# imdea-software/legosnark

Measured on AMD Instinct MI355X. Metric: alt_bn128 G1 MSM point-scalar pairs/s at n=2^20, higher is better.
Workload: dtype u32 limbs (254-bit Montgomery integers)

## Files before the change

legosnark_amd/csrc/msm.hip:

```cpp
#include <hip/hip_runtime.h>
#include <stdint.h>
#include <stdio.h>
#include <stdlib.h>
#include <string.h>
#include <algorithm>
#include <type_traits>
#include <vector>

#include "curves.h"
#include "fp29x2l.h"
#include "fs29.h"
#include "glv.h"
#include "msm.h"
#include "msm_plan.h"

namespace lsa {


template <class F, int K>
__global__ __launch_bounds__(256) void k_normalize(const Jac<F> *__restrict__ in, Aff<F> *__restrict__ out, size_t n) {
    size_t t = (size_t)blockIdx.x * blockDim.x + threadIdx.x;
    size_t base = t * K;
    if (base >= n) return;
    F prod[K];
// ... 258 lines not shown
    const uint32_t *tb = tile_base + ((size_t)k * ntiles + t) * B;
    for (uint32_t x = threadIdx.x; x < B; x += 1024) base[x] = of[x] + tb[x];
    __syncthreads();
    const size_t lo = (size_t)t * SORT_TILE;
    const size_t hi = lo + SORT_TILE < n ? lo + SORT_TILE : n;
    const int32_t *dg = digits + (size_t)k * n;
    const uint16_t *rk = rank + (size_t)k * n;
    for (size_t i = lo + threadIdx.x; i < hi; i += 1024) {
        int32_t sd = dg[i];
        if (sd != 0) {
            uint32_t b = (uint32_t)(sd < 0 ? -sd : sd) - 1;
            uint32_t pt = i < npoints ? (uint32_t)i : ((uint32_t)(i - npoints) | 0x40000000u);
            pt += k * win_stride;
            entries[base[b] + rk[i]] = pt | (sd < 0 ? 0x80000000u : 0u);
        }
    }
}

__global__ __launch_bounds__(1024) void k_tile_scan_rows(const uint16_t *__restrict__ tile_hist, uint32_t Bc, uint32_t R, uint32_t pitch,
                                                         uint32_t *__restrict__ tile_base, uint32_t *__restrict__ hist,
                                                         uint32_t *__restrict__ zero1, uint32_t *__restrict__ zeron, uint32_t nzero) {
    __builtin_amdgcn_s_setprio(3);
    if (blockIdx.x == 0) {
        if (threadIdx.x == 0) *zero1 = 0;
        for (uint32_t x = threadIdx.x; x < nzero; x += 1024) zeron[x] = 0;
    }
    __shared__ uint32_t part[32][33];
    const unsigned lane = threadIdx.x & 63, wv = threadIdx.x >> 6;
    const unsigned bl = lane & 31, grp = 2 * wv + (lane >> 5);
    const uint32_t b = blockIdx.x * 32 + bl;
    const uint32_t per = (R + 31) / 32, r0 = grp * per, r1 = r0 + per < R ? r0 + per : R;
    constexpr uint32_t MAXPER = 16;
    uint32_t v[MAXPER];
    uint32_t sum = 0;
    const bool in_regs = per <= MAXPER;
    if (in_regs) {
#pragma unroll
        for (uint32_t j = 0; j < MAXPER; j++) {
            const uint32_t r = r0 + j;
            v[j] = (b < Bc && r < r1) ? tile_hist[(size_t)r * pitch + b] : 0u;
        }
#pragma unroll
        for (uint32_t j = 0; j < MAXPER; j++) sum += v[j];
    } else if (b < Bc) {
        for (uint32_t r = r0; r < r1; r++) sum += tile_hist[(size_t)r * pitch + b];
    }
    part[grp][bl] = sum;
// ... 152 lines not shown
    const size_t lo = (size_t)t * PART_TILE;
    const uint32_t fine_bits = cm.sh_hi;
    const uint32_t tlow = t & ((1u << (16 - fine_bits)) - 1);
    for (uint32_t j = 0; j < PART_TILE / 1024; j++) {
        const uint32_t il = threadIdx.x + j * 1024;
        const size_t i = lo + il;
        if (i >= n) break;
        const uint32_t seg = segment_of(segs, (uint32_t)i);
        wide_digits(scalars[i], pl, seg * B, [&](unsigned k, int32_t sd) {
            if (sd != 0) {
                const uint32_t b = (uint32_t)(sd < 0 ? -sd : sd) - 1;
                const uint32_t pos = atomicAdd(&lcur[cm.bin(b)], 1u);
                stage[pos] = (tlow << (16 + fine_bits)) | (cm.fine(b) << 16) | (k << 12) | (sd < 0 ? 0x800u : 0u) | il;
            }
        });
    }
    __syncthreads();
    for (uint32_t sg = threadIdx.x >> 5; sg < Bc; sg += 32) {
        const uint32_t a = lstart[sg], e = lstart[sg + 1], g = gdst[sg];
        for (uint32_t x = a + (lane & 31); x < e; x += 32) recs[g + (x - a)] = stage[x];
    }
}

__global__ __launch_bounds__(1024) void k_fine_sort_part(const uint32_t *__restrict__ recs, const uint32_t *__restrict__ offs_c,
                                                         const uint32_t *__restrict__ hist_c, const uint32_t *__restrict__ tile_base,
                                                         uint32_t pitch, uint32_t T, CoarseMap cm, SegList segs, uint32_t win_stride, uint32_t stage_cap,
                                                         uint32_t *__restrict__ entries, uint32_t *__restrict__ hist, uint32_t *__restrict__ offs) {
    __builtin_amdgcn_s_setprio(3);
    extern __shared__ __attribute__((aligned(16))) uint32_t sm[];
    __shared__ uint32_t wsum[16];
    const uint32_t sg = blockIdx.x, lo = offs_c[sg], ns = hist_c[sg];
    const uint32_t fine_bits = cm.sh_hi, FM = 1u << fine_bits, fmask = FM - 1, tbits = 16 - fine_bits;
    const uint32_t F = 1u << cm.bits(sg), bucket0 = cm.first(sg);
    uint32_t *cnt = sm, *cur = sm + FM, *col = sm + 2 * FM, *stage = col + T + 1;
    const unsigned lane = threadIdx.x & 63, wv = threadIdx.x >> 6;
    for (uint32_t x = threadIdx.x; x < F; x += 1024) cnt[x] = 0;
    for (uint32_t x = threadIdx.x; x < T; x += 1024) col[x] = tile_base[(size_t)x * pitch + sg];
    if (threadIdx.x == 0) col[T] = ns;
    auto scan_counters = [&]() {
        const uint32_t per = (F + 1023) >> 10, f0 = threadIdx.x * per;
        uint32_t sum = 0;
        for (uint32_t q = 0; q < per; q++) if (f0 + q < F) sum += cnt[f0 + q];
        uint32_t incl = sum;
#pragma unroll
        for (int d = 1; d < 64; d <<= 1) {
            const uint32_t u = __shfl_up(incl, d, 64);
            if ((int)lane >= d) incl += u;
        }
        if (lane == 63) wsum[wv] = incl;
        __syncthreads();
        uint32_t run = incl - sum;
        for (unsigned w = 0; w < wv; w++) run += wsum[w];
        for (uint32_t q = 0; q < per; q++) {
            if (f0 + q >= F) break;
            const uint32_t c = cnt[f0 + q];
            cur[f0 + q] = run;
            hist[(size_t)bucket0 + f0 + q] = c;
            offs[(size_t)bucket0 + f0 + q] = lo + run;
            run += c;
        }
    };
    auto entry_of = [&](uint32_t r, uint32_t p2) {
        uint32_t a = 0, e = (T + (1u << tbits) - 1) >> tbits;
        while (e - a > 1) {
            const uint32_t m = (a + e) >> 1;
            if (col[m << tbits] <= p2) a = m; else e = m;
        }
        const uint32_t i = ((a << tbits) | (r >> (16 + fine_bits))) * PART_TILE + (r & 0x7ffu);
        const uint32_t local = i - segs.off[segment_of(segs, i)];
        return (local + ((r >> 12) & 15u) * win_stride) | ((r & 0x800u) << 20);
    };
    if (ns <= stage_cap) {
        constexpr uint32_t NR = PART_STAGE / 1024;
        uint32_t r[NR];
#pragma unroll
        for (uint32_t u = 0; u < NR; u++) { const uint32_t p2 = threadIdx.x + u * 1024; r[u] = p2 < ns ? recs[lo + p2] : 0u; }
        __syncthreads();
        uint16_t rk[NR];
#pragma unroll
        for (uint32_t u = 0; u < NR; u++) {
            rk[u] = 0;
            if (threadIdx.x + u * 1024 < ns) rk[u] = (uint16_t)atomicAdd(&cnt[(r[u] >> 16) & fmask], 1u);
        }
        __syncthreads();
        scan_counters();
        __syncthreads();
#pragma unroll
        for (uint32_t u = 0; u < NR; u++) {
            const uint32_t p2 = threadIdx.x + u * 1024;
            if (p2 < ns) stage[cur[(r[u] >> 16) & fmask] + rk[u]] = entry_of(r[u], p2);
        }
        __syncthreads();
        for (uint32_t x = threadIdx.x; x < ns; x += 1024) entries[lo + x] = stage[x];
        return;
    }
    __syncthreads();
    constexpr uint32_t UNR = 8;
    for (uint32_t p0 = threadIdx.x; p0 < ns; p0 += 1024 * UNR) {
        uint32_t r[UNR];
#pragma unroll
        for (uint32_t u = 0; u < UNR; u++) { const uint32_t p2 = p0 + u * 1024; r[u] = p2 < ns ? recs[lo + p2] : 0u; }
#pragma unroll
        for (uint32_t u = 0; u < UNR; u++) if (p0 + u * 1024 < ns) (void)lds_inc_rank(cnt, (r[u] >> 16) & fmask);
    }
    __syncthreads();
    scan_counters();
    __syncthreads();
    for (uint32_t p0 = threadIdx.x; p0 < ns; p0 += 1024 * UNR) {
        uint32_t r[UNR];
#pragma unroll
        for (uint32_t u = 0; u < UNR; u++) { const uint32_t p2 = p0 + u * 1024; r[u] = p2 < ns ? recs[lo + p2] : 0u; }
#pragma unroll
        for (uint32_t u = 0; u < UNR; u++) {
            const uint32_t p2 = p0 + u * 1024;
            if (p2 >= ns) break;
            entries[lo + lds_inc_rank(cur, (r[u] >> 16) & fmask)] = entry_of(r[u], p2);
        }
    }
}

template <class Rec>
struct RecOps;
template <>
struct RecOps<uint64_t> {
    static constexpr uint32_t NF = 128;
    static __device__ __forceinline__ uint32_t fine(uint64_t r) { return (uint32_t)(r >> 32); }
    static __device__ __forceinline__ uint32_t entry(uint64_t r) { return (uint32_t)r; }
};
template <>
struct RecOps<uint32_t> {
// ... 21 lines not shown
        uint32_t incl = tot;
#pragma unroll
        for (int d = 1; d < 64; d <<= 1) {
            uint32_t t = __shfl_up(incl, d, 64);
            if ((int)threadIdx.x >= d) incl += t;
        }
        uint32_t ex = incl - tot;
#pragma unroll
        for (uint32_t q = 0; q < PER; q++) {
            cur[PER * threadIdx.x + q] = ex;
            hist[(size_t)bin * NF + PER * threadIdx.x + q] = c[q];
            offs[(size_t)bin * NF + PER * threadIdx.x + q] = lo + ex;
            ex += c[q];
        }
    }
    __syncthreads();
    for (uint32_t j = threadIdx.x; j < n; j += 1024) {
        const Rec r = recs[lo + j];
        const uint32_t pos = atomicAdd(&cur[O::fine(r)], 1u);
        entries[lo + pos] = O::entry(r);
    }
}

__device__ __forceinline__ uint32_t size_bin(uint32_t cnt, uint32_t bin_shift) { return ((cnt - 1) >> bin_shift) + 1; }
template <class C>
__global__ __launch_bounds__(256) void k_size_hist(const uint32_t *__restrict__ hist, uint32_t nb, uint32_t thr, uint32_t *__restrict__ bin_count,
                                                   uint32_t group_size, uint32_t bin_shift) {
    bin_count += (group_size ? (blockIdx.x * 2048u) / group_size : 0u) * SIZE_BINS;
    __shared__ uint32_t lcnt[SIZE_BINS];
    for (uint32_t t = threadIdx.x; t < SIZE_BINS; t += 256) lcnt[t] = 0;
    __syncthreads();
    const uint32_t base = blockIdx.x * 2048 + threadIdx.x;
#pragma unroll
    for (int j = 0; j < 8; j++) {
        uint32_t g = base + j * 256;
        if (g < nb) { uint32_t cnt = hist[g]; if (cnt > 0 && cnt <= thr) atomicAdd(&lcnt[size_bin(cnt, bin_shift)], 1u); }
    }
    __syncthreads();
    for (uint32_t t = threadIdx.x; t < SIZE_BINS; t += 256) if (lcnt[t]) atomicAdd(&bin_count[t], lcnt[t]);
}
__global__ __launch_bounds__(256) void k_size_scan(const uint32_t *__restrict__ bin_count, uint32_t *__restrict__ bin_start, uint32_t ngroups) {
    __shared__ uint32_t lds[4];
    uint32_t carry = 0;
    for (uint32_t gidx = 0; gidx < ngroups; gidx++) {
        const uint32_t *bc = bin_count + gidx * SIZE_BINS;
        uint32_t *bs = bin_start + gidx * SIZE_BINS;
        uint32_t v[4], s = 0;
#pragma unroll
        for (int j = 0; j < 4; j++) {
            int bin = (int)SIZE_BINS - 1 - (int)(threadIdx.x * 4 + j);
            v[j] = (bin >= 1) ? bc[bin] : 0;
            s += v[j];
        }
        uint32_t tot;
        uint32_t run = carry + block_exclusive_scan_256(s, lds, &tot);
#pragma unroll
        for (int j = 0; j < 4; j++) {
            int bin = (int)SIZE_BINS - 1 - (int)(threadIdx.x * 4 + j);
            if (bin >= 1) bs[bin] = run;
            run += v[j];
        }
        carry += tot;
    }
    if (threadIdx.x == 0) bin_start[0] = carry;
}
template <class C>
__global__ __launch_bounds__(256) void k_size_scatter(const uint32_t *__restrict__ hist, uint32_t nb, uint32_t thr, const uint32_t *__restrict__ bin_start,
                                                      uint32_t *__restrict__ bin_cursor, uint32_t *__restrict__ perm,
                                                      uint32_t *__restrict__ heavy_list, uint32_t *__restrict__ heavy_count,
                                                      typename C::Acc *__restrict__ buckets, uint32_t group_size, uint32_t bin_shift,
                                                      uint32_t split) {
    const uint32_t goff = (group_size ? (blockIdx.x * 2048u) / group_size : 0u) * SIZE_BINS;
    bin_start += goff;
    bin_cursor += goff;
    __shared__ uint32_t lcnt[SIZE_BINS];
    for (uint32_t t = threadIdx.x; t < SIZE_BINS; t += 256) lcnt[t] = 0;
    __syncthreads();
    const uint32_t base = blockIdx.x * 2048 + threadIdx.x;
    uint32_t cnt[8], rank[8];
#pragma unroll
    for (int j = 0; j < 8; j++) {
        uint32_t g = base + j * 256;
        cnt[j] = 0; rank[j] = 0;
        if (g < nb) {
            cnt[j] = hist[g];
            if (cnt[j] == 0) { for (uint32_t h = 0; h < split; h++) buckets[(size_t)g * split + h] = C::inf(); }
            else if (cnt[j] > thr) heavy_list[atomicAdd(heavy_count, 1u)] = g;
            else rank[j] = atomicAdd(&lcnt[size_bin(cnt[j], bin_shift)], 1u);
        }
    }
    __syncthreads();
    for (uint32_t t = threadIdx.x; t < SIZE_BINS; t += 256) {
        uint32_t c = lcnt[t];
        lcnt[t] = c ? atomicAdd(&bin_cursor[t], c) : 0;
    }
    __syncthreads();
#pragma unroll
    for (int j = 0; j < 8; j++) {
        uint32_t g = base + j * 256;
        if (g < nb && cnt[j] > 0 && cnt[j] <= thr) {
            const uint32_t bin = size_bin(cnt[j], bin_shift);
            perm[bin_start[bin] + lcnt[bin] + rank[j]] = g;
        }
    }
}

typedef uint32_t u32x4 __attribute__((ext_vector_type(4)));
template <class B> struct RawBase {
    static_assert(sizeof(B) % 16 == 0, "packed bases are whole 16-byte vectors");
    u32x4 q[sizeof(B) / 16];
};
template <class B>
__device__ __forceinline__ RawBase<B> load_base16(const B *__restrict__ p) {
    const u32x4 *src = reinterpret_cast<const u32x4 *>(p);
    RawBase<B> r;
#pragma unroll
    for (int i = 0; i < (int)(sizeof(B) / 16); i++) r.q[i] = src[i];
    return r;
}
template <class B>
__device__ __forceinline__ B packed_base(RawBase<B> r) {
    B b;
    uint32_t *dst = reinterpret_cast<uint32_t *>(&b);
#pragma unroll
    for (int i = 0; i < (int)(sizeof(B) / 16); i++) {
        asm("" : "+v"(r.q[i]));
// ... 42 lines not shown
            const typename C::Base b0 = packed_base(r0), b1 = packed_base(r1);
            cur = r0;
            if (j + ACC_SPLIT < cnt && C::head_ok(b0, b1)) {
                acc = C::template madd_head<ENDO>(b0, (v >> 31) != 0, ((v >> 30) & 1) != 0, b1, (vn >> 31) != 0, ((vn >> 30) & 1) != 0);
                j += 2 * ACC_SPLIT;
                v = v2;
                vn = v3;
                cur = r2;
            }
        } else {
            cur = base(v);
        }
        for (; j < cnt; j += ACC_SPLIT) {
            const uint32_t vnn = word(j + 2 * ACC_SPLIT);
            const RawBase<typename C::Base> nxt = base(vn);
            acc = C::template madd<ENDO>(acc, packed_base(cur), (v >> 31) != 0, ((v >> 30) & 1) != 0);
            v = vn;
            vn = vnn;
            cur = nxt;
        }
    }
    buckets[(size_t)g * ACC_SPLIT + part] = acc;
}
template <class C, uint32_t ACC_SPLIT>
__global__ __launch_bounds__(256) void k_accumulate(const typename C::Base *__restrict__ bases, const uint32_t *__restrict__ entries,
                                                    const uint32_t *__restrict__ offs, const uint32_t *__restrict__ hist,
                                                    const uint32_t *__restrict__ perm, const uint32_t *__restrict__ nperm,
                                                    typename C::Acc *__restrict__ buckets) {
    accumulate_body<C, ACC_SPLIT>(bases, entries, offs, hist, perm, nperm, buckets);
}
__global__ __launch_bounds__(256) __attribute__((amdgpu_waves_per_eu(2, 2))) void k_accumulate_g2_occ2(
    const CurveG2::Base *__restrict__ bases, const uint32_t *__restrict__ entries, const uint32_t *__restrict__ offs,
    const uint32_t *__restrict__ hist, const uint32_t *__restrict__ perm, const uint32_t *__restrict__ nperm, CurveG2::Acc *__restrict__ buckets) {
    accumulate_body<CurveG2, 1u>(bases, entries, offs, hist, perm, nperm, buckets);
}

__global__ __launch_bounds__(256) void k_accumulate_g2_pair(const AffPackedG2 *__restrict__ bases, const uint32_t *__restrict__ entries,
                                                            const uint32_t *__restrict__ offs, const uint32_t *__restrict__ hist,
                                                            const uint32_t *__restrict__ perm, const uint32_t *__restrict__ nperm,
                                                            XYZZ29x2 *__restrict__ buckets) {
    const uint32_t t = blockIdx.x * blockDim.x + threadIdx.x, pr = t >> 1, part = t & 1;
    if (pr >= *nperm) return;
    const uint32_t g = perm[pr];
    const uint32_t cnt = hist[g];
    const uint32_t *e = entries + offs[g];
    struct Half { uint32_t x[8], y[8]; };
    auto fetch = [&](uint32_t v) {
        const AffPackedG2 &b = bases[v & 0x3fffffffu];
        Half h;
#pragma unroll
        for (int i = 0; i < 8; i++) { h.x[i] = b.w[part][i]; h.y[i] = b.w[2 + part][i]; }
// ... 26 lines not shown
    A r;
    constexpr int NW = sizeof(A) / 4;
    const uint32_t *src = reinterpret_cast<const uint32_t *>(&p);
    uint32_t *dst = reinterpret_cast<uint32_t *>(&r);
#pragma unroll
    for (int i = 0; i < NW; i++) dst[i] = __shfl_down(src[i], delta, 64);
    return r;
}

enum TailKernel { TAIL_HEAVY, TAIL_REDUCE1_LANE, TAIL_REDUCE2_LANE };
template <class C, TailKernel K> struct PairedAdd { static constexpr bool value = false; };
template <> struct PairedAdd<CurveG1, TAIL_HEAVY> { static constexpr bool value = true; };
template <> struct PairedAdd<CurveG1, TAIL_REDUCE1_LANE> { static constexpr bool value = true; };

template <class C, bool PAIRED = false>
__device__ __forceinline__ typename C::Acc wave_sum(typename C::Acc v, unsigned lane) {
    for (unsigned d = 32; d >= 1; d >>= 1) {
        typename C::Acc t = shfl_down_acc(v, d);
        if (lane + d < 64) v = C::template add<PAIRED>(v, t);
    }
    return v;
}

__global__ __launch_bounds__(256) void k_heavy_plan(const uint32_t *__restrict__ hist, const uint32_t *__restrict__ heavy_list,
                                                    const uint32_t *__restrict__ heavy_count, uint32_t *__restrict__ chunk_off) {
    __shared__ uint32_t lds[4];
    __shared__ uint32_t s_chunk;
    const uint32_t nh = *heavy_count;
    uint32_t carry = 0;
    for (uint32_t base = 0; base < nh; base += 256) {
        uint32_t h = base + threadIdx.x;
        uint32_t tot;
        (void)block_exclusive_scan_256(h < nh ? hist[heavy_list[h]] : 0, lds, &tot);
        carry += tot;
    }
    if (threadIdx.x == 0) {
        uint32_t chunk = HEAVY_CHUNK;
        while (chunk < 4096u && carry / (2 * chunk) >= 2048u) chunk *= 2;
        s_chunk = chunk;
    }
    __syncthreads();
    const uint32_t chunk = s_chunk;
    carry = 0;
    for (uint32_t base = 0; base < nh; base += 256) {
        uint32_t h = base + threadIdx.x;
        uint32_t v = h < nh ? (hist[heavy_list[h]] + chunk - 1) / chunk : 0;
        uint32_t tot;
        uint32_t ex = block_exclusive_scan_256(v, lds, &tot);
        if (h < nh) chunk_off[h] = carry + ex;
        carry += tot;
    }
    if (threadIdx.x == 0) { chunk_off[nh] = carry; chunk_off[nh + 1] = chunk; }
}

template <class C>
__global__ __launch_bounds__(64) void k_accumulate_heavy(const typename C::Base *__restrict__ bases, const uint32_t *__restrict__ entries,
                                                         const uint32_t *__restrict__ offs, const uint32_t *__restrict__ hist,
                                                         const uint32_t *__restrict__ heavy_list, const uint32_t *__restrict__ heavy_count,
                                                         const uint32_t *__restrict__ chunk_off, typename C::Acc *__restrict__ partials) {
    const uint32_t nh = *heavy_count;
    if (nh == 0) return;
    const uint32_t total = chunk_off[nh], chunk = chunk_off[nh + 1];
    const unsigned lane = threadIdx.x;
    for (uint32_t v = blockIdx.x; v < total; v += gridDim.x) {
        uint32_t lo = 0, hi = nh;
        while (hi - lo > 1) { uint32_t mid = (lo + hi) >> 1; if (chunk_off[mid] <= v) lo = mid; else hi = mid; }
        const uint32_t g = heavy_list[lo];
        const uint32_t cnt = hist[g];
        const uint32_t start = (v - chunk_off[lo]) * chunk;
        const uint32_t end = start + chunk < cnt ? start + chunk : cnt;
        const uint32_t *e = entries + offs[g];
        typename C::Acc acc = C::inf();
        uint32_t j = start + lane;
        if constexpr (!RotatedLoads<C>::value) {
            for (; j < end; j += 64) {
                uint32_t w = e[j];
                acc = C::madd(acc, bases[w & 0x3fffffffu], (w >> 31) != 0, ((w >> 30) & 1) != 0);
            }
        } else if (j < end) {
            const uint32_t last = j + (end - 1 - j) / 64 * 64;
            auto word = [&](uint32_t k) { return e[k < last ? k : last]; };
            uint32_t w = word(j), wn = word(j + 64);
            RawBase<typename C::Base> cur = load_base16(bases + (w & 0x3fffffffu));
            for (; j < end; j += 64) {
                const uint32_t wnn = word(j + 128);
                const RawBase<typename C::Base> nxt = load_base16(bases + (wn & 0x3fffffffu));
                acc = C::madd(acc, packed_base(cur), (w >> 31) != 0, ((w >> 30) & 1) != 0);
                w = wn;
                wn = wnn;
                cur = nxt;
            }
        }
        acc = wave_sum<C, PairedAdd<C, TAIL_HEAVY>::value>(acc, lane);
        if (lane == 0) partials[v] = acc;
    }
}

template <class C>
__global__ __launch_bounds__(64) void k_heavy_finish(const uint32_t *__restrict__ heavy_list, const uint32_t *__restrict__ heavy_count,
                                                     const uint32_t *__restrict__ chunk_off, const typename C::Acc *__restrict__ partials,
                                                     typename C::Acc *__restrict__ buckets, uint32_t split) {
    const uint32_t nh = *heavy_count;
    unsigned lane = threadIdx.x;
    for (uint32_t h = blockIdx.x; h < nh; h += gridDim.x) {
        typename C::Acc acc = C::inf();
        for (uint32_t v = chunk_off[h] + lane; v < chunk_off[h + 1]; v += 64) acc = C::add(acc, partials[v]);
        acc = wave_sum<C>(acc, lane);
        if (lane == 0) {
            buckets[(size_t)heavy_list[h] * split] = acc;
            for (uint32_t x = 1; x < split; x++) buckets[(size_t)heavy_list[h] * split + x] = C::inf();
        }
    }
}

template <class A>
__device__ __forceinline__ A select_acc(uint32_t mask, const A &a, const A &b) {
    A r;
    const uint32_t *pa = reinterpret_cast<const uint32_t *>(&a), *pb = reinterpret_cast<const uint32_t *>(&b);
    uint32_t *pr = reinterpret_cast<uint32_t *>(&r);
#pragma unroll
    for (int i = 0; i < (int)(sizeof(A) / 4); i++) pr[i] = (pa[i] & mask) | (pb[i] & ~mask);
    return r;
}
template <class A>
__device__ __forceinline__ void quadwave_weighted(A &acc, A &run, unsigned log_mult, unsigned lane) {
    const unsigned q = lane & 3, qi = lane >> 2;
    A s = A::inf();
#pragma unroll 1
    for (unsigned step = 0; step < 9; step++) {
        if (step == 4) {
            s = (qi == 0) ? A::inf() : run;
#pragma unroll 1
            for (unsigned i = 0; i < log_mult; i++) s = quad_dbl(s, q);
        }
// ... 391 lines not shown
    hipLaunchKernelGGL(k_publish, dim3(1), dim3(64), 0, st, (const uint32_t *)nullptr, (uint32_t *)nullptr, 0u);
    for (auto &t : g_tail) if (t.stream) hipLaunchKernelGGL(k_publish, dim3(1), dim3(64), 0, t.stream, (const uint32_t *)nullptr, (uint32_t *)nullptr, 0u);
    HIPCHK(hipDeviceSynchronize());
    return LSA_OK;
}

static int grow_tail_slot(TailBuf &t, size_t bytes) {
    if (bytes <= t.ws.cap) return LSA_OK;
    if (t.pending) HIPCHK(hipEventSynchronize(t.done));
    if (t.ws.ensure(bytes) != 0) { set_error("msm: tail workspace allocation of %zu bytes failed", bytes); return LSA_ERR_NOMEM; }
    return LSA_OK;
}
static int grow_all_tail_slots(size_t bytes) {
    int rc = tail_slots_ready();
    for (auto &t : g_tail) if (!rc) rc = grow_tail_slot(t, bytes);
    return rc;
}
int msm_slot_begin(hipStream_t st, size_t ws_bytes, const void *d_out, MsmSlot *slot, bool inline_tail) {
    int rc = tail_slots_ready();
    if (rc) return rc;
    TailBuf &tb = g_tail[g_slot];
    rc = grow_tail_slot(tb, ws_bytes);
    if (rc) return rc;
    if (tb.pending) HIPCHK(hipStreamWaitEvent(st, tb.done, 0));
    slot->tail = (g_overlap && !inline_tail) ? tb.stream : st;
    slot->ws = tb.ws.ptr;
    slot->aux = tb.aux;
    slot->index = (int)g_slot;
    tb.out = d_out;
    return LSA_OK;
}
static int slot_front_to_tail(TailBuf &tb, hipStream_t tail, hipStream_t st) {
    if (tail == st) return LSA_OK;
    HIPCHK(hipEventRecord(tb.front_done, st));
    HIPCHK(hipStreamWaitEvent(tail, tb.front_done, 0));
    return LSA_OK;
}
static int publish_order_compact(TailBuf &tb, hipStream_t tail) {
    for (auto &o : g_tail) {
        if (&o == &tb || !o.pending || o.out != tb.out) continue;
        if (!o.unjoined && hipEventQuery(o.done) == hipSuccess) { o.pending = false; continue; }
        HIPCHK(hipStreamWaitEvent(tail, o.done, 0));
    }
    return LSA_OK;
}
static int publish_order_large(TailBuf &tb, TailBuf &prev, hipStream_t tail) {
    if (prev.pending && &prev != &tb) HIPCHK(hipStreamWaitEvent(tail, prev.done, 0));
// ... 66 lines not shown
    unsigned blocks = (unsigned)((threads + 255) / 256);
    hipLaunchKernelGGL((k_normalize<F, K>), dim3(blocks), dim3(256), 0, st, d_in, d_out, n);
    HIPCHK(hipGetLastError());
    return LSA_OK;
}
template int normalize_to_affine<Fq>(const Jac<Fq> *, Aff<Fq> *, size_t, hipStream_t);
template int normalize_to_affine<Fq2>(const Jac<Fq2> *, Aff<Fq2> *, size_t, hipStream_t);

static MsmSwitches &switches() {
    static MsmSwitches sw = [] {
        const auto is_one = [](const char *name) { const char *e = getenv(name); return e && e[0] == '1'; };
        MsmSwitches v;
        v.no_rec32 = getenv("LSA_NO_REC32") != nullptr;
        v.no_part = getenv("LSA_NO_PART") != nullptr;
        if (const char *e = getenv("LSA_WIDE_SPLIT")) v.wide_split = (uint32_t)atoi(e);
        v.g2_pair = is_one("LSA_G2_PAIR");
        v.no_reduce_bits = getenv("LSA_NO_REDUCE_BITS") != nullptr;
        v.no_lane_l1 = getenv("LSA_NO_LANE_L1") != nullptr;
        v.g2_lane_l1 = is_one("LSA_G2_LANE_L1");
        if (const char *e = getenv("LSA_WIDE_BIG_MIN")) v.wide_big_min = (size_t)atoll(e);
        return v;
    }();
    return sw;
}
unsigned msm_table_windows(int , size_t n) { return table_copies(n); }

static size_t g_merge_min = 0;
static bool g_merge_min_explicit = false;
void msm_set_merge_min(size_t n) {
    g_merge_min = n;
    g_merge_min_explicit = n != 0;
    switches().table_use_min = n ? n : 1;
}
size_t msm_merge_min() {
    if (g_merge_min == 0) {
        const char *e = getenv("LSA_PRECOMPUTE_MIN");
        g_merge_min = e && atoll(e) > 0 ? (size_t)atoll(e) : (size_t)1 << 19;
    }
    return g_merge_min;
}
bool msm_merge_min_is_explicit() { return g_merge_min_explicit; }
bool msm_uses_table(size_t n) { return n >= switches().table_use_min; }

template <class C>
__global__ __launch_bounds__(256) void k_shift_window(const typename C::Base *__restrict__ prev, Jac<typename C::Field> *__restrict__ out,
                                                      size_t n, unsigned c) {
// ... 81 lines not shown
        res = tws + p.tail[T_RES];
    }
};

struct Marks {
    hipEvent_t *ev;
    void operator()(int i, hipStream_t s) const { if (ev) (void)hipEventRecord(ev[i], s); }
};

template <class C>
static void launch_sort(const PipelinePlan &p, const MsmBuffers<typename C::Acc> &b, const Fr *d_scalars, const SegList &segs, hipStream_t st,
                        const Marks &mark) {
    const size_t n = p.n;
    if (p.wide) {
        hipLaunchKernelGGL(k_hist_wide, dim3(p.wtiles), dim3(1024), p.lds_hist_wide, st, d_scalars, n, segs, p.pl, p.B, p.Bc, p.cm, p.pitch, p.wtile, b.tile_hist);
        mark(1, st);
        hipLaunchKernelGGL(k_tile_scan_rows, dim3((p.Bc + 31) / 32), dim3(1024), 0, st, b.tile_hist, p.Bc, p.wtiles, p.pitch, b.tile_base, b.hist_c, b.heavy_count,
                           b.bin_count, (uint32_t)(3 * SIZE_BINS));
        mark(2, st);
        if (p.part) {
            hipLaunchKernelGGL(k_partition, dim3(p.wtiles), dim3(1024), p.lds_partition, st, d_scalars, n, segs, p.pl, p.B, p.Bc, p.cm, p.pitch,
                               b.tile_hist, b.hist_c, b.offs_c, b.tile_base, (uint32_t *)b.recs);
            hipLaunchKernelGGL(k_fine_sort_part, dim3(p.Bc), dim3(1024), p.lds_fine_sort_part, st, (const uint32_t *)b.recs, b.offs_c, b.hist_c,
                               b.tile_base, p.pitch, p.wtiles, p.cm, segs, p.win_stride, p.stage_cap, b.entries, b.hist, b.offs);
        } else if (p.rec32) {
            hipLaunchKernelGGL(k_scatter_wide<2>, dim3(p.wtiles), dim3(1024), p.lds_scatter_wide, st, d_scalars, n, segs, p.pl, p.B, p.Bc, p.pitch, p.wtile, b.hist_c, b.offs_c, b.tile_base, b.recs, p.win_stride);
            hipLaunchKernelGGL(k_fine_sort<uint32_t>, dim3(p.Bc), dim3(1024), 0, st, (const uint32_t *)b.recs, b.offs_c, b.hist_c, b.entries, b.hist, b.offs);
        } else if (p.fine) {
            hipLaunchKernelGGL(k_scatter_wide<1>, dim3(p.wtiles), dim3(1024), p.lds_scatter_wide, st, d_scalars, n, segs, p.pl, p.B, p.Bc, p.pitch, p.wtile, b.hist_c, b.offs_c, b.tile_base, b.recs, p.win_stride);
            hipLaunchKernelGGL(k_fine_sort<uint64_t>, dim3(p.Bc), dim3(1024), 0, st, (const uint64_t *)b.recs, b.offs_c, b.hist_c, b.entries, b.hist, b.offs);
        } else {
            hipLaunchKernelGGL(k_scatter_wide<0>, dim3(p.wtiles), dim3(1024), p.lds_scatter_wide, st, d_scalars, n, segs, p.pl, p.B, p.Bc, p.pitch, p.wtile, b.hist_c, b.offs_c, b.tile_base, (void *)b.entries, p.win_stride);
        }
        mark(3, st);
    } else {
        hipLaunchKernelGGL((k_digits<C::GLV>), dim3((unsigned)((n + 255) / 256)), dim3(256), 0, st, d_scalars, n, p.c, p.nwin, b.digits);
        hipLaunchKernelGGL(k_rank, dim3(p.ntiles, p.nwin), dim3(1024), p.lds_rank, st, b.digits, p.nv, p.B, p.ntiles, b.rank, b.tile_hist, 0u);
        hipLaunchKernelGGL(k_tile_scan, dim3((p.nb + 255) / 256), dim3(256), 0, st, b.tile_hist, p.B, p.ntiles, p.nb, b.tile_base, b.hist);
        mark(1, st);
        hipLaunchKernelGGL(k_scan_sums, dim3(p.scan_blocks), dim3(256), 0, st, b.hist, p.nb, b.bsum);
        hipLaunchKernelGGL(k_scan_blocks, dim3(1), dim3(256), 0, st, b.bsum, p.scan_blocks);
        hipLaunchKernelGGL(k_scan_final, dim3(p.scan_blocks), dim3(256), 0, st, b.hist, b.bsum, p.nb, b.offs);
        mark(2, st);
        hipLaunchKernelGGL(k_scatter, dim3(p.ntiles, p.nwin), dim3(1024), p.lds_scatter, st, b.digits, b.rank, b.offs, b.tile_base, p.nv, n, p.B, p.ntiles, b.entries, 0u);
        mark(3, st);
    }
}

template <class C>
static int launch_accumulate(const PipelinePlan &p, const MsmBuffers<typename C::Acc> &b, const typename C::Base *d_bases, hipStream_t st, const Marks &mark) {
    constexpr bool g2 = std::is_same<C, CurveG2>::value;
    if (!p.wide || p.reuse_sort) {
        HIPCHK(hipMemsetAsync(b.heavy_count, 0, 4, st));
        HIPCHK(hipMemsetAsync(b.bin_count, 0, (size_t)3 * SIZE_BINS * 4, st));
    }
    const unsigned sb = (p.nb + 2047) / 2048;
    const uint32_t gsz = 0u, ngroups = 1;
    hipLaunchKernelGGL((k_size_hist<C>), dim3(sb), dim3(256), 0, st, b.hist, p.nb, p.heavy_threshold, b.bin_count, gsz, p.bin_shift);
    hipLaunchKernelGGL(k_size_scan, dim3(1), dim3(256), 0, st, b.bin_count, b.bin_start, ngroups);
    hipLaunchKernelGGL((k_size_scatter<C>), dim3(sb), dim3(256), 0, st, b.hist, p.nb, p.heavy_threshold, b.bin_start, b.bin_cursor, b.perm, b.heavy_list, b.heavy_count, b.buckets, gsz, p.bin_shift, p.split);
    mark(4, st);
    const dim3 one_lane((p.nb + 255) / 256), two_lanes((p.nb * 2 + 255) / 256);
    if (g2 && p.g2_pair) {
        if constexpr (g2) hipLaunchKernelGGL(k_accumulate_g2_pair, two_lanes, dim3(256), 0, st, d_bases, b.entries, b.offs, b.hist, b.perm, b.bin_start, b.buckets);
    } else if (g2 && p.split == 1) {
        if constexpr (g2) hipLaunchKernelGGL(k_accumulate_g2_occ2, one_lane, dim3(256), 0, st, d_bases, b.entries, b.offs, b.hist, b.perm, b.bin_start, b.buckets);
    } else if (p.split == 1) {
        hipLaunchKernelGGL((k_accumulate<C, 1u>), one_lane, dim3(256), 0, st, d_bases, b.entries, b.offs, b.hist, b.perm, b.bin_start, b.buckets);
    } else {
        hipLaunchKernelGGL((k_accumulate<C, 2u>), two_lanes, dim3(256), 0, st, d_bases, b.entries, b.offs, b.hist, b.perm, b.bin_start, b.buckets);
    }
    hipLaunchKernelGGL(k_heavy_plan, dim3(1), dim3(256), 0, st, b.hist, b.heavy_list, b.heavy_count, b.chunk_off);
    hipLaunchKernelGGL((k_accumulate_heavy<C>), dim3(4096), dim3(64), 0, st, d_bases, b.entries, b.offs, b.hist,
                       b.heavy_list, b.heavy_count, b.chunk_off, b.hpart);
    hipLaunchKernelGGL((k_heavy_finish<C>), dim3(256), dim3(64), 0, st, b.heavy_list, b.heavy_count, b.chunk_off, b.hpart, b.buckets, p.split);
    mark(5, st);
    return LSA_OK;
}

template <class C>
static int launch_tail(const PipelinePlan &p, const MsmBuffers<typename C::Acc> &b, Jac<typename C::Field> *d_out, hipStream_t tail, bool inline_tail,
                       bool lane_l1, TailBuf &tb, TailBuf &prev, const Marks &mark) {
    using A = typename C::Acc;
    using J = Jac<typename C::Field>;
    constexpr bool g1 = std::is_same<C, CurveG1>::value;
    if (p.big)
        hipLaunchKernelGGL((k_reduce1_lane<C>), dim3(p.kw * ((p.T + 63) / 64)), dim3(64), 0, tail, b.buckets, p.B, p.L, p.split, b.wave_out);
    else
        hipLaunchKernelGGL((k_reduce1<C>), dim3(p.kw * p.wpw), dim3(64), 0, tail, b.buckets, p.B, p.L, p.logL, p.wpw, p.split, b.wave_out);
    A *lvl_in = b.wave_out, *lvl_out = b.window_sums;
    uint32_t m = p.wpw, lm = p.big ? p.logL : p.logL + 4;
    J *res = inline_tail ? d_out : (J *)b.res;
    const auto level = [&](bool lane) {
        const uint32_t m_out = (m + 15) / 16;
        if (lane) hipLaunchKernelGGL((k_reduce2_lane<C>), dim3((m_out + 63) / 64), dim3(64), 0, tail, lvl_in, m, m_out, lm, lvl_out);
        else hipLaunchKernelGGL((k_reduce2<C>), dim3(p.kw * m_out), dim3(64), 0, tail, lvl_in, m, m_out, lm, lvl_out);
        std::swap(lvl_in, lvl_out);
        m = m_out;
// ... 158 lines not shown
```

Measured before the change: 834.3 million.

## Fuse size-binning and heavy-bucket planning into sort and accumulate kernels

Bucket-size histogram counting moves into the fine-sort kernel. The size scan is folded into each size-scatter block, and the last block to finish, chosen with a grid-wide ticket, builds the heavy-bucket chunk plan. Heavy-bucket accumulation now runs in extra blocks appended to the G1 accumulate grid, and the last chunk of each bucket does the final reduction using atomic tickets and release/acquire fences. Together these remove several small serial kernel launches (size_hist, size_scan, heavy_plan, heavy_finish) from the critical path, at the cost of cross-block synchronisation complexity. A host-side event query also skips a stream wait when the tail slot has already finished.

```diff
diff --git a/legosnark_amd/csrc/msm.hip b/legosnark_amd/csrc/msm.hip
--- a/legosnark_amd/csrc/msm.hip
+++ b/legosnark_amd/csrc/msm.hip
@@ -304,7 +304,7 @@
                                                          uint32_t *__restrict__ zero1, uint32_t *__restrict__ zeron, uint32_t nzero) {
     __builtin_amdgcn_s_setprio(3);
     if (blockIdx.x == 0) {
-        if (threadIdx.x == 0) *zero1 = 0;
+        if (threadIdx.x < 2) zero1[threadIdx.x] = 0;
         for (uint32_t x = threadIdx.x; x < nzero; x += 1024) zeron[x] = 0;
     }
     __shared__ uint32_t part[32][33];
@@ -503,13 +503,22 @@
     }
 }
 
+__device__ __forceinline__ uint32_t size_bin(uint32_t cnt, uint32_t bin_shift) { return ((cnt - 1) >> bin_shift) + 1; }
+
 __global__ __launch_bounds__(1024) void k_fine_sort_part(const uint32_t *__restrict__ recs, const uint32_t *__restrict__ offs_c,
                                                          const uint32_t *__restrict__ hist_c, const uint32_t *__restrict__ tile_base,
                                                          uint32_t pitch, uint32_t T, CoarseMap cm, SegList segs, uint32_t win_stride, uint32_t stage_cap,
-                                                         uint32_t *__restrict__ entries, uint32_t *__restrict__ hist, uint32_t *__restrict__ offs) {
+                                                         uint32_t *__restrict__ entries, uint32_t *__restrict__ hist, uint32_t *__restrict__ offs,
+                                                         uint32_t *__restrict__ bin_count, uint32_t thr, uint32_t bin_shift) {
     __builtin_amdgcn_s_setprio(3);
     extern __shared__ __attribute__((aligned(16))) uint32_t sm[];
     __shared__ uint32_t wsum[16];
+    __shared__ uint32_t lbin[SIZE_BINS];
+    for (uint32_t x = threadIdx.x; x < SIZE_BINS; x += 1024) lbin[x] = 0;
+    const auto flush_bins = [&]() {
+        if (!bin_count) return;
+        for (uint32_t x = threadIdx.x; x < SIZE_BINS; x += 1024) if (lbin[x]) atomicAdd(&bin_count[x], lbin[x]);
+    };
     const uint32_t sg = blockIdx.x, lo = offs_c[sg], ns = hist_c[sg];
     const uint32_t fine_bits = cm.sh_hi, FM = 1u << fine_bits, fmask = FM - 1, tbits = 16 - fine_bits;
     const uint32_t F = 1u << cm.bits(sg), bucket0 = cm.first(sg);
@@ -539,6 +548,7 @@
             hist[(size_t)bucket0 + f0 + q] = c;
             offs[(size_t)bucket0 + f0 + q] = lo + run;
             run += c;
+            if (bin_count && c > 0 && c <= thr) atomicAdd(&lbin[size_bin(c, bin_shift)], 1u);
         }
     };
     auto entry_of = [&](uint32_t r, uint32_t p2) {
@@ -566,6 +576,7 @@
         __syncthreads();
         scan_counters();
         __syncthreads();
+        flush_bins();
 #pragma unroll
         for (uint32_t u = 0; u < NR; u++) {
             const uint32_t p2 = threadIdx.x + u * 1024;
@@ -587,6 +598,7 @@
     __syncthreads();
     scan_counters();
     __syncthreads();
+    flush_bins();
     for (uint32_t p0 = threadIdx.x; p0 < ns; p0 += 1024 * UNR) {
         uint32_t r[UNR];
 #pragma unroll
@@ -654,11 +666,9 @@
     }
 }
 
-__device__ __forceinline__ uint32_t size_bin(uint32_t cnt, uint32_t bin_shift) { return ((cnt - 1) >> bin_shift) + 1; }
 template <class C>
 __global__ __launch_bounds__(256) void k_size_hist(const uint32_t *__restrict__ hist, uint32_t nb, uint32_t thr, uint32_t *__restrict__ bin_count,
-                                                   uint32_t group_size, uint32_t bin_shift) {
-    bin_count += (group_size ? (blockIdx.x * 2048u) / group_size : 0u) * SIZE_BINS;
+                                                   uint32_t bin_shift) {
     __shared__ uint32_t lcnt[SIZE_BINS];
     for (uint32_t t = threadIdx.x; t < SIZE_BINS; t += 256) lcnt[t] = 0;
     __syncthreads();
@@ -671,45 +681,82 @@
     __syncthreads();
     for (uint32_t t = threadIdx.x; t < SIZE_BINS; t += 256) if (lcnt[t]) atomicAdd(&bin_count[t], lcnt[t]);
 }
-__global__ __launch_bounds__(256) void k_size_scan(const uint32_t *__restrict__ bin_count, uint32_t *__restrict__ bin_start, uint32_t ngroups) {
+__device__ __forceinline__ uint32_t size_scan_256(const uint32_t *__restrict__ bin_count, uint32_t *start, uint32_t *lds) {
+    uint32_t v[4], s = 0;
+#pragma unroll
+    for (int j = 0; j < 4; j++) {
+        int bin = (int)SIZE_BINS - 1 - (int)(threadIdx.x * 4 + j);
+        v[j] = (bin >= 1) ? bin_count[bin] : 0;
+        s += v[j];
+    }
+    uint32_t tot;
+    uint32_t run = block_exclusive_scan_256(s, lds, &tot);
+#pragma unroll
+    for (int j = 0; j < 4; j++) {
+        int bin = (int)SIZE_BINS - 1 - (int)(threadIdx.x * 4 + j);
+        if (bin >= 1) start[bin] = run;
+        run += v[j];
+    }
+    return tot;
+}
+__global__ __launch_bounds__(256) void k_size_scan(const uint32_t *__restrict__ bin_count, uint32_t *__restrict__ bin_start) {
     __shared__ uint32_t lds[4];
+    const uint32_t tot = size_scan_256(bin_count, bin_start, lds);
+    if (threadIdx.x == 0) bin_start[0] = tot;
+}
+
+__device__ __forceinline__ uint32_t load_agent(const uint32_t *p) { return __hip_atomic_load(p, __ATOMIC_RELAXED, __HIP_MEMORY_SCOPE_AGENT); }
+
+__device__ __forceinline__ void heavy_plan_256(const uint32_t *__restrict__ hist, const uint32_t *heavy_list, uint32_t nh,
+                                               uint32_t *__restrict__ chunk_off, uint32_t *ticket_end, uint32_t *lds, uint32_t *s_chunk) {
     uint32_t carry = 0;
-    for (uint32_t gidx = 0; gidx < ngroups; gidx++) {
-        const uint32_t *bc = bin_count + gidx * SIZE_BINS;
-        uint32_t *bs = bin_start + gidx * SIZE_BINS;
-        uint32_t v[4], s = 0;
-#pragma unroll
-        for (int j = 0; j < 4; j++) {
-            int bin = (int)SIZE_BINS - 1 - (int)(threadIdx.x * 4 + j);
-            v[j] = (bin >= 1) ? bc[bin] : 0;
-            s += v[j];
-        }
+    for (uint32_t base = 0; base < nh; base += 256) {
+        uint32_t h = base + threadIdx.x;
         uint32_t tot;
-        uint32_t run = carry + block_exclusive_scan_256(s, lds, &tot);
-#pragma unroll
-        for (int j = 0; j < 4; j++) {
-            int bin = (int)SIZE_BINS - 1 - (int)(threadIdx.x * 4 + j);
-            if (bin >= 1) bs[bin] = run;
-            run += v[j];
-        }
+        (void)block_exclusive_scan_256(h < nh ? hist[load_agent(heavy_list + h)] : 0, lds, &tot);
         carry += tot;
     }
-    if (threadIdx.x == 0) bin_start[0] = carry;
-}
-template <class C>
-__global__ __launch_bounds__(256) void k_size_scatter(const uint32_t *__restrict__ hist, uint32_t nb, uint32_t thr, const uint32_t *__restrict__ bin_start,
-                                                      uint32_t *__restrict__ bin_cursor, uint32_t *__restrict__ perm,
-                                                      uint32_t *__restrict__ heavy_list, uint32_t *__restrict__ heavy_count,
-                                                      typename C::Acc *__restrict__ buckets, uint32_t group_size, uint32_t bin_shift,
-                                                      uint32_t split) {
-    const uint32_t goff = (group_size ? (blockIdx.x * 2048u) / group_size : 0u) * SIZE_BINS;
-    bin_start += goff;
-    bin_cursor += goff;
+    if (threadIdx.x == 0) {
+        uint32_t chunk = HEAVY_CHUNK;
+        while (chunk < 4096u && carry / (2 * chunk) >= 2048u) chunk *= 2;
+        *s_chunk = chunk;
+    }
+    __syncthreads();
+    const uint32_t chunk = *s_chunk;
+    carry = 0;
+    for (uint32_t base = 0; base < nh; base += 256) {
+        uint32_t h = base + threadIdx.x;
+        uint32_t v = h < nh ? (hist[load_agent(heavy_list + h)] + chunk - 1) / chunk : 0;
+        uint32_t tot;
+        uint32_t ex = block_exclusive_scan_256(v, lds, &tot);
+        if (h < nh) {
+            chunk_off[h] = carry + ex;
+            if (ticket_end) ticket_end[-1 - (ptrdiff_t)h] = 0;
+        }
+        carry += tot;
+    }
+    if (threadIdx.x == 0) { chunk_off[nh] = carry; chunk_off[nh + 1] = chunk; }
+}
+
+template <class C, bool FUSED>
+__global__ __launch_bounds__(256) void k_size_scatter(const uint32_t *__restrict__ hist, uint32_t nb, uint32_t thr, const uint32_t *__restrict__ bin_count,
+                                                      uint32_t *__restrict__ bin_start, uint32_t *__restrict__ bin_cursor, uint32_t *perm,
+                                                      uint32_t *heavy_list, uint32_t *heavy_count,
+                                                      typename C::Acc *__restrict__ buckets, uint32_t bin_shift, uint32_t split,
+                                                      uint32_t *__restrict__ chunk_off) {
     __shared__ uint32_t lcnt[SIZE_BINS];
+    __shared__ uint32_t lstart[FUSED ? SIZE_BINS : 1];
+    __shared__ uint32_t lds[4];
+    __shared__ uint32_t s_word;
     for (uint32_t t = threadIdx.x; t < SIZE_BINS; t += 256) lcnt[t] = 0;
+    if constexpr (FUSED) {
+        const uint32_t tot = size_scan_256(bin_count, lstart, lds);
+        if (blockIdx.x == 0 && threadIdx.x == 0) bin_start[0] = tot;
+    }
     __syncthreads();
     const uint32_t base = blockIdx.x * 2048 + threadIdx.x;
     uint32_t cnt[8], rank[8];
+    int wrote_heavy = 0;
 #pragma unroll
     for (int j = 0; j < 8; j++) {
         uint32_t g = base + j * 256;
@@ -717,7 +764,7 @@
         if (g < nb) {
             cnt[j] = hist[g];
             if (cnt[j] == 0) { for (uint32_t h = 0; h < split; h++) buckets[(size_t)g * split + h] = C::inf(); }
-            else if (cnt[j] > thr) heavy_list[atomicAdd(heavy_count, 1u)] = g;
+            else if (cnt[j] > thr) { heavy_list[atomicAdd(heavy_count, 1u)] = g; wrote_heavy = 1; }
             else rank[j] = atomicAdd(&lcnt[size_bin(cnt[j], bin_shift)], 1u);
         }
     }
@@ -732,8 +779,20 @@
         uint32_t g = base + j * 256;
         if (g < nb && cnt[j] > 0 && cnt[j] <= thr) {
             const uint32_t bin = size_bin(cnt[j], bin_shift);
-            perm[bin_start[bin] + lcnt[bin] + rank[j]] = g;
-        }
+            perm[(FUSED ? lstart[bin] : bin_start[bin]) + lcnt[bin] + rank[j]] = g;
+        }
+    }
+    if constexpr (FUSED) {
+        const bool wrote = __syncthreads_or(wrote_heavy);
+        if (threadIdx.x == 0) {
+            if (wrote) __builtin_amdgcn_fence(__ATOMIC_RELEASE, "agent");
+            s_word = atomicAdd(heavy_count + 1, 1u);
+        }
+        __syncthreads();
+        if (s_word != gridDim.x - 1) return;
+        __builtin_amdgcn_fence(__ATOMIC_ACQUIRE, "agent");
+        __syncthreads();
+        heavy_plan_256(hist, heavy_list, load_agent(heavy_count), chunk_off, perm + nb, lds, &s_word);
     }
 }
 
@@ -822,11 +881,33 @@
     }
     buckets[(size_t)g * ACC_SPLIT + part] = acc;
 }
+template <class A>
+struct HeavyArgs {
+    const uint32_t *heavy_list, *heavy_count, *chunk_off;
+    uint32_t *ticket_end;
+    A *partials;
+    uint32_t split, blocks;
+};
+template <class C>
+__device__ __forceinline__ void heavy_body(const typename C::Base *__restrict__ bases, const uint32_t *__restrict__ entries,
+                                           const uint32_t *__restrict__ offs, const uint32_t *__restrict__ hist,
+                                           const HeavyArgs<typename C::Acc> &hv, typename C::Acc *__restrict__ buckets,
+                                           uint32_t wave, uint32_t nwaves, unsigned lane);
+template <class C> struct HeavyRides { static constexpr bool value = false; };
+template <> struct HeavyRides<CurveG1> { static constexpr bool value = true; };
+constexpr uint32_t HEAVY_RIDE_BLOCKS = 1024;
 template <class C, uint32_t ACC_SPLIT>
 __global__ __launch_bounds__(256) void k_accumulate(const typename C::Base *__restrict__ bases, const uint32_t *__restrict__ entries,
                                                     const uint32_t *__restrict__ offs, const uint32_t *__restrict__ hist,
                                                     const uint32_t *__restrict__ perm, const uint32_t *__restrict__ nperm,
-                                                    typename C::Acc *__restrict__ buckets) {
+                                                    typename C::Acc *__restrict__ buckets, HeavyArgs<typename C::Acc> hv) {
+    if constexpr (HeavyRides<C>::value) {
+        const uint32_t own = gridDim.x - hv.blocks;
+        if (blockIdx.x >= own) {
+            heavy_body<C>(bases, entries, offs, hist, hv, buckets, (blockIdx.x - own) * 4 + (threadIdx.x >> 6), hv.blocks * 4, threadIdx.x & 63);
+            return;
+        }
+    }
     accumulate_body<C, ACC_SPLIT>(bases, entries, offs, hist, perm, nperm, buckets);
 }
 __global__ __launch_bounds__(256) __attribute__((amdgpu_waves_per_eu(2, 2))) void k_accumulate_g2_occ2(
@@ -899,37 +980,102 @@
     return v;
 }
 
+
+template <class C>
+__device__ __forceinline__ typename C::Acc heavy_chunk_sum(const typename C::Base *__restrict__ bases, const uint32_t *__restrict__ e,
+                                                           uint32_t start, uint32_t end, unsigned lane) {
+    typename C::Acc acc = C::inf();
+    uint32_t j = start + lane;
+    if constexpr (!RotatedLoads<C>::value) {
+        for (; j < end; j += 64) {
+            uint32_t w = e[j];
+            acc = C::madd(acc, bases[w & 0x3fffffffu], (w >> 31) != 0, ((w >> 30) & 1) != 0);
+        }
+    } else if (j < end) {
+        const uint32_t last = j + (end - 1 - j) / 64 * 64;
+        auto word = [&](uint32_t k) { return e[k < last ? k : last]; };
+        uint32_t w = word(j), wn = word(j + 64);
+        RawBase<typename C::Base> cur = load_base16(bases + (w & 0x3fffffffu));
+        for (; j < end; j += 64) {
+            const uint32_t wnn = word(j + 128);
+            const RawBase<typename C::Base> nxt = load_base16(bases + (wn & 0x3fffffffu));
+            acc = C::madd(acc, packed_base(cur), (w >> 31) != 0, ((w >> 30) & 1) != 0);
+            w = wn;
+            wn = wnn;
+            cur = nxt;
+        }
+    }
+    return wave_sum<C, PairedAdd<C, TAIL_HEAVY>::value>(acc, lane);
+}
+template <class C, bool AGENT>
+__device__ __forceinline__ typename C::Acc heavy_bucket_sum(const uint32_t *__restrict__ chunk_off, const typename C::Acc *partials, uint32_t h, unsigned lane) {
+    typename C::Acc acc = C::inf();
+    for (uint32_t v = chunk_off[h] + lane; v < chunk_off[h + 1]; v += 64) {
+        typename C::Acc t;
+        if constexpr (AGENT) {
+            const uint32_t *src = reinterpret_cast<const uint32_t *>(partials + v);
+            uint32_t *dst = reinterpret_cast<uint32_t *>(&t);
+#pragma unroll
+            for (int i = 0; i < (int)(sizeof(t) / 4); i++) dst[i] = load_agent(src + i);
+        } else {
+            t = partials[v];
+        }
+        acc = C::add(acc, t);
+    }
+    return wave_sum<C>(acc, lane);
+}
+template <class C>
+__device__ __forceinline__ void heavy_store(typename C::Acc *__restrict__ buckets, uint32_t g, uint32_t split, const typename C::Acc &acc) {
+    buckets[(size_t)g * split] = acc;
+    for (uint32_t x = 1; x < split; x++) buckets[(size_t)g * split + x] = C::inf();
+}
+
+template <class C>
+__device__ __forceinline__ void heavy_body(const typename C::Base *__restrict__ bases, const uint32_t *__restrict__ entries,
+                                           const uint32_t *__restrict__ offs, const uint32_t *__restrict__ hist,
+                                           const HeavyArgs<typename C::Acc> &hv, typename C::Acc *__restrict__ buckets,
+                                           uint32_t wave, uint32_t nwaves, unsigned lane) {
+    const uint32_t nh = *hv.heavy_count;
+    if (nh == 0) return;
+    const uint32_t *__restrict__ heavy_list = hv.heavy_list, *__restrict__ chunk_off = hv.chunk_off;
+    uint32_t *ticket_end = hv.ticket_end;
+    typename C::Acc *partials = hv.partials;
+    const uint32_t split = hv.split;
+    const uint32_t total = chunk_off[nh], chunk = chunk_off[nh + 1];
+    for (uint32_t v = wave; v < total; v += nwaves) {
+        uint32_t lo = 0, hi = nh;
+        while (hi - lo > 1) { uint32_t mid = (lo + hi) >> 1; if (chunk_off[mid] <= v) lo = mid; else hi = mid; }
+        const uint32_t g = heavy_list[lo];
+        const uint32_t cnt = hist[g];
+        const uint32_t start = (v - chunk_off[lo]) * chunk;
+        const uint32_t end = start + chunk < cnt ? start + chunk : cnt;
+        const typename C::Acc part = heavy_chunk_sum<C>(bases, entries + offs[g], start, end, lane);
+        uint32_t arrived = 0;
+        if (lane == 0) {
+            partials[v] = part;
+            __builtin_amdgcn_fence(__ATOMIC_RELEASE, "agent");
+            arrived = atomicAdd(ticket_end - 1 - (ptrdiff_t)lo, 1u);
+        }
+        arrived = __builtin_amdgcn_readfirstlane(arrived);
+        if (arrived + 1 != chunk_off[lo + 1] - chunk_off[lo]) continue;
+        __builtin_amdgcn_fence(__ATOMIC_ACQUIRE, "agent");
+        const typename C::Acc acc = heavy_bucket_sum<C, true>(chunk_off, partials, lo, lane);
+        if (lane == 0) heavy_store<C>(buckets, g, split, acc);
+    }
+}
+template <class C>
+__global__ __launch_bounds__(64) void k_heavy(const typename C::Base *__restrict__ bases, const uint32_t *__restrict__ entries,
+                                              const uint32_t *__restrict__ offs, const uint32_t *__restrict__ hist,
+                                              HeavyArgs<typename C::Acc> hv, typename C::Acc *__restrict__ buckets) {
+    heavy_body<C>(bases, entries, offs, hist, hv, buckets, blockIdx.x, gridDim.x, threadIdx.x);
+}
+
 __global__ __launch_bounds__(256) void k_heavy_plan(const uint32_t *__restrict__ hist, const uint32_t *__restrict__ heavy_list,
                                                     const uint32_t *__restrict__ heavy_count, uint32_t *__restrict__ chunk_off) {
     __shared__ uint32_t lds[4];
     __shared__ uint32_t s_chunk;
-    const uint32_t nh = *heavy_count;
-    uint32_t carry = 0;
-    for (uint32_t base = 0; base < nh; base += 256) {
-        uint32_t h = base + threadIdx.x;
-        uint32_t tot;
-        (void)block_exclusive_scan_256(h < nh ? hist[heavy_list[h]] : 0, lds, &tot);
-        carry += tot;
-    }
-    if (threadIdx.x == 0) {
-        uint32_t chunk = HEAVY_CHUNK;
-        while (chunk < 4096u && carry / (2 * chunk) >= 2048u) chunk *= 2;
-        s_chunk = chunk;
-    }
-    __syncthreads();
-    const uint32_t chunk = s_chunk;
-    carry = 0;
-    for (uint32_t base = 0; base < nh; base += 256) {
-        uint32_t h = base + threadIdx.x;
-        uint32_t v = h < nh ? (hist[heavy_list[h]] + chunk - 1) / chunk : 0;
-        uint32_t tot;
-        uint32_t ex = block_exclusive_scan_256(v, lds, &tot);
-        if (h < nh) chunk_off[h] = carry + ex;
-        carry += tot;
-    }
-    if (threadIdx.x == 0) { chunk_off[nh] = carry; chunk_off[nh + 1] = chunk; }
-}
-
+    heavy_plan_256(hist, heavy_list, *heavy_count, chunk_off, nullptr, lds, &s_chunk);
+}
 template <class C>
 __global__ __launch_bounds__(64) void k_accumulate_heavy(const typename C::Base *__restrict__ bases, const uint32_t *__restrict__ entries,
                                                          const uint32_t *__restrict__ offs, const uint32_t *__restrict__ hist,
@@ -946,33 +1092,10 @@
         const uint32_t cnt = hist[g];
         const uint32_t start = (v - chunk_off[lo]) * chunk;
         const uint32_t end = start + chunk < cnt ? start + chunk : cnt;
-        const uint32_t *e = entries + offs[g];
-        typename C::Acc acc = C::inf();
-        uint32_t j = start + lane;
-        if constexpr (!RotatedLoads<C>::value) {
-            for (; j < end; j += 64) {
-                uint32_t w = e[j];
-                acc = C::madd(acc, bases[w & 0x3fffffffu], (w >> 31) != 0, ((w >> 30) & 1) != 0);
-            }
-        } else if (j < end) {
-            const uint32_t last = j + (end - 1 - j) / 64 * 64;
-            auto word = [&](uint32_t k) { return e[k < last ? k : last]; };
-            uint32_t w = word(j), wn = word(j + 64);
-            RawBase<typename C::Base> cur = load_base16(bases + (w & 0x3fffffffu));
-            for (; j < end; j += 64) {
-                const uint32_t wnn = word(j + 128);
-                const RawBase<typename C::Base> nxt = load_base16(bases + (wn & 0x3fffffffu));
-                acc = C::madd(acc, packed_base(cur), (w >> 31) != 0, ((w >> 30) & 1) != 0);
-                w = wn;
-                wn = wnn;
-                cur = nxt;
-            }
-        }
-        acc = wave_sum<C, PairedAdd<C, TAIL_HEAVY>::value>(acc, lane);
+        const typename C::Acc acc = heavy_chunk_sum<C>(bases, entries + offs[g], start, end, lane);
         if (lane == 0) partials[v] = acc;
     }
 }
-
 template <class C>
 __global__ __launch_bounds__(64) void k_heavy_finish(const uint32_t *__restrict__ heavy_list, const uint32_t *__restrict__ heavy_count,
                                                      const uint32_t *__restrict__ chunk_off, const typename C::Acc *__restrict__ partials,
@@ -980,13 +1103,8 @@
     const uint32_t nh = *heavy_count;
     unsigned lane = threadIdx.x;
     for (uint32_t h = blockIdx.x; h < nh; h += gridDim.x) {
-        typename C::Acc acc = C::inf();
-        for (uint32_t v = chunk_off[h] + lane; v < chunk_off[h + 1]; v += 64) acc = C::add(acc, partials[v]);
-        acc = wave_sum<C>(acc, lane);
-        if (lane == 0) {
-            buckets[(size_t)heavy_list[h] * split] = acc;
-            for (uint32_t x = 1; x < split; x++) buckets[(size_t)heavy_list[h] * split + x] = C::inf();
-        }
+        const typename C::Acc acc = heavy_bucket_sum<C, false>(chunk_off, partials, h, lane);
+        if (lane == 0) heavy_store<C>(buckets, heavy_list[h], split, acc);
     }
 }
 
@@ -1424,7 +1542,14 @@
     TailBuf &tb = g_tail[g_slot];
     rc = grow_tail_slot(tb, ws_bytes);
     if (rc) return rc;
-    if (tb.pending) HIPCHK(hipStreamWaitEvent(st, tb.done, 0));
+    if (tb.pending) {
+        bool done = false;
+        if (!tb.unjoined) {
+            done = hipEventQuery(tb.done) == hipSuccess;
+            if (!done) (void)hipGetLastError();
+        }
+        if (!done) HIPCHK(hipStreamWaitEvent(st, tb.done, 0));
+    }
     slot->tail = (g_overlap && !inline_tail) ? tb.stream : st;
     slot->ws = tb.ws.ptr;
     slot->aux = tb.aux;
@@ -1537,6 +1662,10 @@
         return v;
     }();
     return sw;
+}
+static bool front_legacy() {
+    static const bool v = [] { const char *e = getenv("LSA_FRONT_LEGACY"); return e && e[0] == '1'; }();
+    return v;
 }
 unsigned msm_table_windows(int , size_t n) { return table_copies(n); }
 
@@ -1664,7 +1793,8 @@
             hipLaunchKernelGGL(k_partition, dim3(p.wtiles), dim3(1024), p.lds_partition, st, d_scalars, n, segs, p.pl, p.B, p.Bc, p.cm, p.pitch,
                                b.tile_hist, b.hist_c, b.offs_c, b.tile_base, (uint32_t *)b.recs);
             hipLaunchKernelGGL(k_fine_sort_part, dim3(p.Bc), dim3(1024), p.lds_fine_sort_part, st, (const uint32_t *)b.recs, b.offs_c, b.hist_c,
-                               b.tile_base, p.pitch, p.wtiles, p.cm, segs, p.win_stride, p.stage_cap, b.entries, b.hist, b.offs);
+                               b.tile_base, p.pitch, p.wtiles, p.cm, segs, p.win_stride, p.stage_cap, b.entries, b.hist, b.offs,
+                               front_legacy() ? nullptr : b.bin_count, p.heavy_threshold, p.bin_shift);
         } else if (p.rec32) {
             hipLaunchKernelGGL(k_scatter_wide<2>, dim3(p.wtiles), dim3(1024), p.lds_scatter_wide, st, d_scalars, n, segs, p.pl, p.B, p.Bc, p.pitch, p.wtile, b.hist_c, b.offs_c, b.tile_base, b.recs, p.win_stride);
             hipLaunchKernelGGL(k_fine_sort<uint32_t>, dim3(p.Bc), dim3(1024), 0, st, (const uint32_t *)b.recs, b.offs_c, b.hist_c, b.entries, b.hist, b.offs);
@@ -1693,29 +1823,41 @@
 static int launch_accumulate(const PipelinePlan &p, const MsmBuffers<typename C::Acc> &b, const typename C::Base *d_bases, hipStream_t st, const Marks &mark) {
     constexpr bool g2 = std::is_same<C, CurveG2>::value;
     if (!p.wide || p.reuse_sort) {
-        HIPCHK(hipMemsetAsync(b.heavy_count, 0, 4, st));
+        HIPCHK(hipMemsetAsync(b.heavy_count, 0, 8, st));
         HIPCHK(hipMemsetAsync(b.bin_count, 0, (size_t)3 * SIZE_BINS * 4, st));
     }
+    const bool legacy = front_legacy();
     const unsigned sb = (p.nb + 2047) / 2048;
-    const uint32_t gsz = 0u, ngroups = 1;
-    hipLaunchKernelGGL((k_size_hist<C>), dim3(sb), dim3(256), 0, st, b.hist, p.nb, p.heavy_threshold, b.bin_count, gsz, p.bin_shift);
-    hipLaunchKernelGGL(k_size_scan, dim3(1), dim3(256), 0, st, b.bin_count, b.bin_start, ngroups);
-    hipLaunchKernelGGL((k_size_scatter<C>), dim3(sb), dim3(256), 0, st, b.hist, p.nb, p.heavy_threshold, b.bin_start, b.bin_cursor, b.perm, b.heavy_list, b.heavy_count, b.buckets, gsz, p.bin_shift, p.split);
+    if (legacy || !(p.wide && p.part) || p.reuse_sort)
+        hipLaunchKernelGGL((k_size_hist<C>), dim3(sb), dim3(256), 0, st, b.hist, p.nb, p.heavy_threshold, b.bin_count, p.bin_shift);
+    if (legacy) {
+        hipLaunchKernelGGL(k_size_scan, dim3(1), dim3(256), 0, st, b.bin_count, b.bin_start);
+        hipLaunchKernelGGL((k_size_scatter<C, false>), dim3(sb), dim3(256), 0, st, b.hist, p.nb, p.heavy_threshold, b.bin_count, b.bin_start, b.bin_cursor, b.perm,
+                           b.heavy_list, b.heavy_count, b.buckets, p.bin_shift, p.split, b.chunk_off);
+    } else {
+        hipLaunchKernelGGL((k_size_scatter<C, true>), dim3(sb), dim3(256), 0, st, b.hist, p.nb, p.heavy_threshold, b.bin_count, b.bin_start, b.bin_cursor, b.perm,
+                           b.heavy_list, b.heavy_count, b.buckets, p.bin_shift, p.split, b.chunk_off);
+    }
     mark(4, st);
-    const dim3 one_lane((p.nb + 255) / 256), two_lanes((p.nb * 2 + 255) / 256);
+    const bool rides = !legacy && HeavyRides<C>::value;
+    const HeavyArgs<typename C::Acc> hv = {b.heavy_list, b.heavy_count, b.chunk_off, b.perm + p.nb, b.hpart, p.split, rides ? HEAVY_RIDE_BLOCKS : 0u};
+    if (!legacy && !rides) hipLaunchKernelGGL((k_heavy<C>), dim3(4096), dim3(64), 0, st, d_bases, b.entries, b.offs, b.hist, hv, b.buckets);
+    const dim3 one_lane((p.nb + 255) / 256 + hv.blocks), two_lanes((p.nb * 2 + 255) / 256 + hv.blocks);
     if (g2 && p.g2_pair) {
         if constexpr (g2) hipLaunchKernelGGL(k_accumulate_g2_pair, two_lanes, dim3(256), 0, st, d_bases, b.entries, b.offs, b.hist, b.perm, b.bin_start, b.buckets);
     } else if (g2 && p.split == 1) {
         if constexpr (g2) hipLaunchKernelGGL(k_accumulate_g2_occ2, one_lane, dim3(256), 0, st, d_bases, b.entries, b.offs, b.hist, b.perm, b.bin_start, b.buckets);
     } else if (p.split == 1) {
-        hipLaunchKernelGGL((k_accumulate<C, 1u>), one_lane, dim3(256), 0, st, d_bases, b.entries, b.offs, b.hist, b.perm, b.bin_start, b.buckets);
+        hipLaunchKernelGGL((k_accumulate<C, 1u>), one_lane, dim3(256), 0, st, d_bases, b.entries, b.offs, b.hist, b.perm, b.bin_start, b.buckets, hv);
     } else {
-        hipLaunchKernelGGL((k_accumulate<C, 2u>), two_lanes, dim3(256), 0, st, d_bases, b.entries, b.offs, b.hist, b.perm, b.bin_start, b.buckets);
-    }
-    hipLaunchKernelGGL(k_heavy_plan, dim3(1), dim3(256), 0, st, b.hist, b.heavy_list, b.heavy_count, b.chunk_off);
-    hipLaunchKernelGGL((k_accumulate_heavy<C>), dim3(4096), dim3(64), 0, st, d_bases, b.entries, b.offs, b.hist,
-                       b.heavy_list, b.heavy_count, b.chunk_off, b.hpart);
-    hipLaunchKernelGGL((k_heavy_finish<C>), dim3(256), dim3(64), 0, st, b.heavy_list, b.heavy_count, b.chunk_off, b.hpart, b.buckets, p.split);
+        hipLaunchKernelGGL((k_accumulate<C, 2u>), two_lanes, dim3(256), 0, st, d_bases, b.entries, b.offs, b.hist, b.perm, b.bin_start, b.buckets, hv);
+    }
+    if (legacy) {
+        hipLaunchKernelGGL(k_heavy_plan, dim3(1), dim3(256), 0, st, b.hist, b.heavy_list, b.heavy_count, b.chunk_off);
+        hipLaunchKernelGGL((k_accumulate_heavy<C>), dim3(4096), dim3(64), 0, st, d_bases, b.entries, b.offs, b.hist,
+                           b.heavy_list, b.heavy_count, b.chunk_off, b.hpart);
+        hipLaunchKernelGGL((k_heavy_finish<C>), dim3(256), dim3(64), 0, st, b.heavy_list, b.heavy_count, b.chunk_off, b.hpart, b.buckets, p.split);
+    }
     mark(5, st);
     return LSA_OK;
 }
```

Result: no change. 833.5 million (-0.1%).
